# imalexlee/simple-vk-renderer

Measured on AMD Instinct MI355X. Metric: shaded fragments/s, higher is better.
Workload: dtype f32

## Files before the change

### simple-vk-renderer_amd/csrc/k_image.hip

```cpp
#include <hip/hip_fp16.h>

#include "svr_launch.h"

namespace svr {

__global__ __launch_bounds__(256) void fill16f_kernel(uint4* dst, uint32_t n_vec, uint32_t n_pixels, uint2 px, const uint32_t* poison) {
  if (*poison) return;
  for (uint32_t i = blockIdx.x * blockDim.x + threadIdx.x; i < n_vec; i += gridDim.x * blockDim.x)
    dst[i] = make_uint4(px.x, px.y, px.x, px.y);
  if (blockIdx.x == 0 && threadIdx.x == 0 && (n_pixels & 1u))
    reinterpret_cast<uint2*>(dst)[n_pixels - 1] = px;
}
__global__ __launch_bounds__(256) void fill8_kernel(uint32_t* dst, uint32_t n_pixels, uint32_t px, const uint32_t* poison) {
  if (*poison) return;
  uint32_t n_vec = n_pixels >> 2;
  uint4* d4 = reinterpret_cast<uint4*>(dst);
  for (uint32_t i = blockIdx.x * blockDim.x + threadIdx.x; i < n_vec; i += gridDim.x * blockDim.x)
    d4[i] = make_uint4(px, px, px, px);
  if (blockIdx.x == 0 && threadIdx.x < (n_pixels & 3u)) dst[(n_vec << 2) + threadIdx.x] = px;
}

static inline uint32_t stream_grid(uint32_t n_items) {
  uint32_t g = (n_items + 255u) / 256u;
  return g < 1u ? 1u : (g > 2048u ? 2048u : g);
}

void launch_fill_color(void* color, uint32_t n_pixels, int color_format, uint64_t packed_pixel, const uint32_t* poison,
                       hipStream_t s) {
  if (color_format == SVR_COLOR_RGBA16F) {
    uint2 px = make_uint2((uint32_t)packed_pixel, (uint32_t)(packed_pixel >> 32));
    uint32_t n_vec = n_pixels >> 1;
    hipLaunchKernelGGL(fill16f_kernel, dim3(stream_grid(n_vec)), dim3(256), 0, s, (uint4*)color, n_vec, n_pixels, px, poison);
  } else {
    hipLaunchKernelGGL(fill8_kernel, dim3(stream_grid(n_pixels >> 2)), dim3(256), 0, s, (uint32_t*)color, n_pixels,
                       (uint32_t)packed_pixel, poison);
  }
}

__global__ __launch_bounds__(256) void downsample_kernel(const uint32_t* src, uint32_t sw, uint32_t sh, uint32_t* dst,
                                                         uint32_t dw, uint32_t dh) {
  uint32_t idx = blockIdx.x * blockDim.x + threadIdx.x;
  if (idx >= dw * dh) return;
  uint32_t i = idx % dw, j = idx / dw;
  long long nx = (long long)(2u * i + 1u) * sw - dw, dx = 2ll * dw;
  long long ny = (long long)(2u * j + 1u) * sh - dh, dy = 2ll * dh;
  long long i0 = nx >= 0 ? nx / dx : -((-nx + dx - 1) / dx);
  long long j0 = ny >= 0 ? ny / dy : -((-ny + dy - 1) / dy);
  long long wx1 = nx - i0 * dx, wx0 = dx - wx1;
  long long wy1 = ny - j0 * dy, wy0 = dy - wy1;
  long long i1 = i0 + 1, j1 = j0 + 1;
  i0 = min(max(i0, 0ll), (long long)sw - 1);
  i1 = min(max(i1, 0ll), (long long)sw - 1);
  j0 = min(max(j0, 0ll), (long long)sh - 1);
  j1 = min(max(j1, 0ll), (long long)sh - 1);
  uint32_t t00 = src[j0 * sw + i0], t10 = src[j0 * sw + i1], t01 = src[j1 * sw + i0], t11 = src[j1 * sw + i1];
  long long den = dx * dy;
  uint32_t out = 0;
#pragma unroll
  for (int c = 0; c < 4; c++) {
    long long a = (t00 >> (8 * c)) & 0xffu, b = (t10 >> (8 * c)) & 0xffu;
    long long cc = (t01 >> (8 * c)) & 0xffu, d = (t11 >> (8 * c)) & 0xffu;
    long long num = wy0 * (wx0 * a + wx1 * b) + wy1 * (wx0 * cc + wx1 * d);
    long long q = num / den, r = num - q * den;
    if (2 * r > den || (2 * r == den && (q & 1))) q++;
    out |= (uint32_t)q << (8 * c);
  }
  dst[idx] = out;
}

void launch_downsample(const uint8_t* src, uint32_t sw, uint32_t sh, uint8_t* dst, uint32_t dw, uint32_t dh,
                       hipStream_t s) {
  uint32_t n = dw * dh;
  hipLaunchKernelGGL(downsample_kernel, dim3((n + 255u) / 256u), dim3(256), 0, s, (const uint32_t*)src, sw, sh,
                     (uint32_t*)dst, dw, dh);
}

__device__ __forceinline__ uint32_t h2un8(uint32_t hbits) {
  float f = __half2float(__ushort_as_half((unsigned short)hbits));
  return (uint32_t)__float2int_rn(fminf(fmaxf(f, 0.0f), 1.0f) * 255.0f);
}
__global__ __launch_bounds__(256) void cvt16f_to_8_kernel(const uint2* src, uint32_t* dst, uint32_t n_pixels) {
  for (uint32_t i = blockIdx.x * blockDim.x + threadIdx.x; i < n_pixels; i += gridDim.x * blockDim.x) {
    uint2 p = src[i];
    dst[i] = h2un8(p.x & 0xffffu) | (h2un8(p.x >> 16) << 8) | (h2un8(p.y & 0xffffu) << 16) | (h2un8(p.y >> 16) << 24);
  }
}
__device__ __forceinline__ float pin32(float x) {
  asm volatile("" : "+v"(x));
  return x;
}
__device__ __forceinline__ void store_target(void* color, int fmt, size_t p, float r, float g, float b, float a) {
  if (fmt == SVR_COLOR_RGBA16F) {
    r = pin32(r); g = pin32(g); b = pin32(b); a = pin32(a);
    uint32_t hr = __half_as_ushort(__float2half_rn(r)), hg = __half_as_ushort(__float2half_rn(g));
    uint32_t hb = __half_as_ushort(__float2half_rn(b)), ha = __half_as_ushort(__float2half_rn(a));
    reinterpret_cast<uint2*>(color)[p] = make_uint2(hr | (hg << 16), hb | (ha << 16));
  } else {
    auto un8 = [](float f) { return (uint32_t)__float2int_rn(fminf(fmaxf(f, 0.0f), 1.0f) * 255.0f); };
    reinterpret_cast<uint32_t*>(color)[p] = un8(r) | (un8(g) << 8) | (un8(b) << 16) | (un8(a) << 24);
  }
}

__device__ __forceinline__ float sky_cos(float x) {
  const float kTwoOverPi = 0x1.45f306p-1f, kPio2Hi = 0x1.921fb6p+0f, kPio2Mid = -0x1.777a5cp-25f, kPio2Lo = -0x1.ee59dap-50f;
  float k = rintf(x * kTwoOverPi);
  float r = fmaf(-k, kPio2Hi, x);
  r = fmaf(-k, kPio2Mid, r);
  r = fmaf(-k, kPio2Lo, r);
  float z = r * r;
  float sn = fmaf(fmaf(fmaf(-1.9515295891e-4f, z, 8.3321608736e-3f), z, -1.6666654611e-1f) * z, r, r);
  float cs = fmaf(fmaf(fmaf(2.443315711809948e-5f, z, -1.388731625493765e-3f), z, 4.166664568298827e-2f) * z, z,
                  fmaf(-0.5f, z, 1.0f));
  int q = (int)k & 3;
  float v = (q & 1) ? sn : cs;
  return (q == 1 || q == 2) ? -v : v;
}
__device__ __forceinline__ float sky_fract(float a) { return a - floorf(a); }
__device__ __forceinline__ float sky_noisy_star(float x, float y, float thr) {
  float s = sky_fract(415.92653f * (sky_cos(x * 37.0f) + sky_cos(y * 57.0f)));
  if (!(s >= thr)) return 0.0f;
  float t = (s - thr) / (1.0f - thr);
  float t2 = t * t, t4 = t2 * t2;
  return t4 * t2;
}

struct BackgroundData {
  float d[16];
};
__global__ __launch_bounds__(256) void background_kernel(void* color, int fmt, uint32_t W, uint32_t H, uint32_t y_first,
                                                         uint32_t n_rows, int effect, BackgroundData pc, const uint32_t* poison) {
  if (*poison) return;
  const float fh = (float)H;
  const uint32_t n = W * n_rows;
  for (uint32_t i = blockIdx.x * blockDim.x + threadIdx.x; i < n; i += gridDim.x * blockDim.x) {
    uint32_t x = i % W, y = y_first + i / W;
    float r, g, b, a;
    if (effect == SVR_BACKGROUND_GRADIENT) {
      float blend = (float)y / fh, inv = 1.0f - blend;
      r = fmaf(pc.d[4], blend, pc.d[0] * inv);
      g = fmaf(pc.d[5], blend, pc.d[1] * inv);
      b = fmaf(pc.d[6], blend, pc.d[2] * inv);
      a = fmaf(pc.d[7], blend, pc.d[3] * inv);
    } else {
      float fx = (float)x, fy = (float)y, thr = pc.d[3];
      float sx = fx + 0.2f, sy = fy + -0.06f;
      float frx = sky_fract(sx), fry = sky_fract(sy), gx = floorf(sx), gy = floorf(sy);
      float v1 = sky_noisy_star(gx, gy, thr), v2 = sky_noisy_star(gx, gy + 1.0f, thr);
      float v3 = sky_noisy_star(gx + 1.0f, gy, thr), v4 = sky_noisy_star(gx + 1.0f, gy + 1.0f, thr);
      float star = (v1 * (1.0f - frx)) * (1.0f - fry);
      star = fmaf(v2 * (1.0f - frx), fry, star);
      star = fmaf(v3 * frx, 1.0f - fry, star);
      star = fmaf(v4 * frx, fry, star);
      r = (pc.d[0] * fy) / fh + star;
      g = (pc.d[1] * fy) / fh + star;
      b = (pc.d[2] * fy) / fh + star;
      a = 1.0f;
    }
// ... 109 lines not shown
```

### simple-vk-renderer_amd/csrc/k_tile.hip

```cpp
#include <hip/hip_fp16.h>

#include <hip/hip_ext.h>

#include <cstdlib>
#include <type_traits>

#include "svr_launch.h"

namespace svr {

constexpr uint32_t REC_COMMON = 0x80000000u;
#ifndef SVR_PRIO_COST
#define SVR_PRIO_COST 200u
#endif
constexpr int BATCH = 64;
constexpr uint32_t SREC = 7;

constexpr float kInv255 = 0x1.010102p-8f;
constexpr float kG0 = 0x1.c51282p-2f, kG1 = -0x1.14a3a2p-2f, kG2 = 0x1.37536ap-3f, kG3 = -0x1.778474p-5f;

__device__ __forceinline__ float lod_from_rho2(float rho2) {
  uint32_t bits = f2u(rho2);
  int e = (int)(bits >> 23) - 127;
  float m = u2f((bits & 0x7fffffu) | 0x3f800000u);
  float t = m - 1.0f;
  float g = fmaf(fmaf(fmaf(kG3, t, kG2), t, kG1), t, kG0);
  float s = t * (1.0f - t);
  float l = fmaf(s, g, t);
  float lam = 0.5f * ((float)e + l);
  lam = (rho2 <= 0x1p+100f) ? lam : 50.0f;
  lam = (rho2 >= 0x1p-100f) ? lam : -50.0f;
  return lam;
}

__device__ __forceinline__ float lerpf(float a, float b, float t) { return fmaf(t, b - a, a); }

struct TexD {
  uint32_t base_off;
  uint32_t w, h, lw, lh, levels, filters;
  float min_lod, max_lod;
};

struct Taps {
  uint32_t o00, o10, o01, o11;
  float alpha, beta;
};
template <bool POW2 = false>
__device__ __forceinline__ Taps level_taps(int wl, int hl, uint32_t base, bool linear, float u, float v) {
  float U = (u - floorf(u)) * (float)wl;
  float V = (v - floorf(v)) * (float)hl;
  float Uh = U - 0.5f, Vh = V - 0.5f;
  float fu = floorf(linear ? Uh : U), fv = floorf(linear ? Vh : V);
  Taps tp;
  tp.alpha = linear ? Uh - fu : 0.0f;
  tp.beta = linear ? Vh - fv : 0.0f;
  int i0 = (int)fu, j0 = (int)fv;
  int i1 = linear ? i0 + 1 : i0, j1 = linear ? j0 + 1 : j0;
  if (POW2) {
    i0 &= wl - 1;
    i1 &= wl - 1;
    j0 &= hl - 1;
    j1 &= hl - 1;
  } else {
    if (i0 < 0) i0 += wl;
    if (i0 >= wl) i0 -= wl;
    if (i1 >= wl) i1 -= wl;
    if (j0 < 0) j0 += hl;
    if (j0 >= hl) j0 -= hl;
    if (j1 >= hl) j1 -= hl;
  }
  const uint32_t r0 = __umul24((uint32_t)j0, (uint32_t)wl), r1 = __umul24((uint32_t)j1, (uint32_t)wl);
  tp.o00 = base + (r0 + (uint32_t)i0) * 4u;
  tp.o10 = base + (r0 + (uint32_t)i1) * 4u;
  tp.o01 = base + (r1 + (uint32_t)i0) * 4u;
  tp.o11 = base + (r1 + (uint32_t)i1) * 4u;
  return tp;
}
__device__ __forceinline__ uint32_t texel(const uint8_t* arena, uint32_t off) {
  return *reinterpret_cast<const uint32_t*>(arena + off);
}
__device__ __forceinline__ float chan(uint32_t t, int c) { return (float)((t >> (8 * c)) & 0xffu) * kInv255; }
__device__ __forceinline__ float bilerp(uint32_t t00, uint32_t t10, uint32_t t01, uint32_t t11, int c, float a, float b) {
  return lerpf(lerpf(chan(t00, c), chan(t10, c), a), lerpf(chan(t01, c), chan(t11, c), a), b);
}

__device__ __forceinline__ float interp3(float a0, float da1, float da2, float b1, float b2, float r) {
  return fmaf(b2, da2, fmaf(b1, da1, a0)) * r;
}

struct FragAttr {
  float b1, b2, r, u, v, nx, ny, nz, light, cr, cg, cb, won;
};

__device__ __forceinline__ float quad_partner_x(float v) { return u2f((uint32_t)__builtin_amdgcn_mov_dpp((int)f2u(v), 0xB1, 0xf, 0xf, true)); }
__device__ __forceinline__ float quad_partner_y(float v) { return u2f((uint32_t)__builtin_amdgcn_mov_dpp((int)f2u(v), 0x128, 0xf, 0xf, true)); }
template <bool TRACE, bool COMMON = false, bool ATTR = false>
__device__ __forceinline__ float4 shade_pixel(const FrameParams& P, uint32_t rec, int px, int py, float* trace, const bool quads = false,
                                              FragAttr* fa = nullptr) {
  const TriRec* tr = P.recs + rec;
  const uint4* q4 = reinterpret_cast<const uint4*>(tr);
  const float4* f4 = reinterpret_cast<const float4*>(tr);
  const double2* d2 = reinterpret_cast<const double2*>(tr);
  uint4 hdr = q4[0];
  float4 zrow = f4[1];
  double2 c2 = d2[2], c3 = d2[3], c4 = d2[4], c5 = d2[5], c6 = d2[6];
  uint4 td = q4[7];
  float4 s0 = f4[8], s1 = f4[9], s2 = f4[10], s3 = f4[11], s4 = f4[12], s5 = f4[13], s6 = f4[14];
  uint32_t flags = hdr.w;
  float inv_area = zrow.w;
  double A1, B1, A2, B2, e1, e2;
  double C1 = c5.y, C2 = c6.x;
  A1 = c2.y; B1 = c4.x; A2 = c3.x; B2 = c4.y;
  double dx = (double)px, dy = (double)py;
  e1 = fma(A1, dx, fma(B1, dy, C1)) + ((flags & F_T1) ? 1.0 : 0.0);
  e2 = fma(A2, dx, fma(B2, dy, C2)) + ((flags & F_T2) ? 1.0 : 0.0);
  TexD t;
  t.base_off = (uint32_t)(unsigned long long)__double_as_longlong(c6.y);
  t.w = td.x & 0xffffu;
  t.h = td.x >> 16;
  t.lw = td.y & 0xffu;
  t.lh = (td.y >> 8) & 0xffu;
  t.levels = (td.y >> 16) & 0xffu;
  t.filters = td.y >> 24;
  t.min_lod = u2f(td.z);
  t.max_lod = u2f(td.w);
  float b1 = (float)e1 * inv_area, b2 = (float)e2 * inv_area;
  float q0 = s0.x, dq1 = s0.y, dq2 = s0.z;
  const float qq = fmaf(b2, dq2, fmaf(b1, dq1, q0));
  float hb1 = 0.0f, hb2 = 0.0f, vb1 = 0.0f, vb2 = 0.0f, hq = 1.0f, vq = 1.0f;
  if (!quads) {
    double sxp = (px & 1) ? -1.0 : 1.0, syp = (py & 1) ? -1.0 : 1.0;
    hb1 = (float)fma(sxp, A1, e1) * inv_area, hb2 = (float)fma(sxp, A2, e2) * inv_area;
    vb1 = (float)fma(syp, B1, e1) * inv_area, vb2 = (float)fma(syp, B2, e2) * inv_area;
    hq = fmaf(hb2, dq2, fmaf(hb1, dq1, q0)), vq = fmaf(vb2, dq2, fmaf(vb1, dq1, q0));
  }
  float r, hr = 0.0f, vr = 0.0f;
  if (COMMON && !quads) {
    rcp3_ieee(qq, hq, vq, r, hr, vr);
  } else {
    r = rcp_ieee(qq);
  }
  const uint32_t kind = COMMON ? (uint32_t)PIPE_MESH : ((flags >> F_KIND_SHIFT) & 3u);
  float cr = interp3(s1.z, s3.z, s5.z, b1, b2, r);
  float cg = interp3(s1.w, s3.w, s5.w, b1, b2, r);
  float cb = interp3(s2.x, s4.x, s6.x, b1, b2, r);
  if (ATTR) { fa->b1 = b1; fa->b2 = b2; fa->r = r; fa->won = 1.0f; }
  if (kind == PIPE_COLORED_TRIANGLE) return make_float4(cr, cg, cb, 1.0f);
  float u = interp3(s2.y, s4.y, s6.y, b1, b2, r), v = interp3(s2.z, s4.z, s6.z, b1, b2, r);
  if (ATTR) { fa->u = u; fa->v = v; }
  if (!COMMON) {
    hr = rcp_ieee(hq);
    vr = rcp_ieee(vq);
  }
  float uh, vh, uv_, vv_;
  if (quads) {
    uh = quad_partner_x(u), vh = quad_partner_x(v);
    uv_ = quad_partner_y(u), vv_ = quad_partner_y(v);
  } else {
    uh = interp3(s2.y, s4.y, s6.y, hb1, hb2, hr), vh = interp3(s2.z, s4.z, s6.z, hb1, hb2, hr);
    uv_ = interp3(s2.y, s4.y, s6.y, vb1, vb2, vr), vv_ = interp3(s2.z, s4.z, s6.z, vb1, vb2, vr);
  }
  float dudx = (px & 1) ? (u - uh) : (uh - u);
  float dvdx = (px & 1) ? (v - vh) : (vh - v);
  float dudy = (py & 1) ? (u - uv_) : (uv_ - u);
  float dvdy = (py & 1) ? (v - vv_) : (vv_ - v);
  float W0 = (float)t.w, H0 = (float)t.h;
  float mx = dudx * W0, my = dvdx * H0;
  float nx_ = dudy * W0, ny_ = dvdy * H0;
  float rho2 = fmaxf(fmaf(mx, mx, my * my), fmaf(nx_, nx_, ny_ * ny_));
  float lambda = fminf(fmaxf(lod_from_rho2(rho2), t.min_lod), t.max_lod);
  const bool linear = COMMON ? true : (((lambda <= 0.0f) ? (t.filters & 1u) : ((t.filters >> 1) & 1u)) != 0u);
  int q = (int)t.levels - 1;
  const bool mip_linear = COMMON ? true : (((t.filters >> 2) & 1u) != 0u);
  int dn = min(max((int)ceilf(lambda + 0.5f) - 1, 0), q);
  float lc = fminf(fmaxf(lambda, 0.0f), (float)q);
  float fl = floorf(lc);
  int dhi = mip_linear ? (int)fl : dn;
  float delta = mip_linear ? lc - fl : 0.0f;
  int dlo = mip_linear ? min(dhi + 1, q) : dn;
  float us = (fabsf(u) < 8388608.0f) ? u : 0.0f, vs = (fabsf(v) < 8388608.0f) ? v : 0.0f;
  const int whi = (int)max(t.w >> dhi, 1u), hhi = (int)max(t.h >> dhi, 1u);
  const uint32_t bhi = t.base_off + mip_offset(t.lw, t.lh, (uint32_t)dhi);
  Taps th = level_taps<COMMON>(whi, hhi, bhi, linear, us, vs);
  const uint8_t* tb = P.tex_arena;
  uint32_t h00 = texel(tb, th.o00), h10 = texel(tb, th.o10), h01 = texel(tb, th.o01), h11 = texel(tb, th.o11);
  const bool two_levels = __any(delta != 0.0f);
  Taps tl = th;
  uint32_t l00 = 0, l10 = 0, l01 = 0, l11 = 0;
  if (two_levels) {
    const int wlo = (int)max(t.w >> dlo, 1u), hlo = (int)max(t.h >> dlo, 1u);
    const uint32_t step = 4u << ((uint32_t)max((int)t.lw - dhi, 0) + (uint32_t)max((int)t.lh - dhi, 0));
    const uint32_t blo = dlo != dhi ? bhi + step : bhi;
    tl = level_taps<COMMON>(wlo, hlo, blo, linear, us, vs);
    l00 = texel(tb, tl.o00);
    l10 = texel(tb, tl.o10);
    l01 = texel(tb, tl.o01);
    l11 = texel(tb, tl.o11);
  }
  float4 tx;
  tx.x = bilerp(h00, h10, h01, h11, 0, th.alpha, th.beta);
  tx.y = bilerp(h00, h10, h01, h11, 1, th.alpha, th.beta);
  tx.z = bilerp(h00, h10, h01, h11, 2, th.alpha, th.beta);
  tx.w = 1.0f;
  if (two_levels) {
    tx.x = lerpf(tx.x, bilerp(l00, l10, l01, l11, 0, tl.alpha, tl.beta), delta);
    tx.y = lerpf(tx.y, bilerp(l00, l10, l01, l11, 1, tl.alpha, tl.beta), delta);
    tx.z = lerpf(tx.z, bilerp(l00, l10, l01, l11, 2, tl.alpha, tl.beta), delta);
  }
  if (TRACE) {
    trace[0] = (float)(hdr.z >> 2); trace[1] = b1; trace[2] = b2; trace[3] = r; trace[4] = u; trace[5] = v;
    trace[6] = dudx; trace[7] = dvdx; trace[8] = dudy; trace[9] = dvdy; trace[10] = lambda;
    trace[11] = tx.x; trace[12] = tx.y; trace[13] = tx.z;
    trace[26] = hb1; trace[27] = hb2; trace[28] = vb1; trace[29] = vb2; trace[30] = hr; trace[31] = vr;
  }
  if (kind == PIPE_TEX_IMAGE) {
    tx.w = bilerp(h00, h10, h01, h11, 3, th.alpha, th.beta);
    if (two_levels) tx.w = lerpf(tx.w, bilerp(l00, l10, l01, l11, 3, tl.alpha, tl.beta), delta);
    return tx;
  }
  float nx = interp3(s0.w, s2.w, s4.w, b1, b2, r);
  float ny = interp3(s1.x, s3.x, s5.x, b1, b2, r);
  float nz = interp3(s1.y, s3.y, s5.y, b1, b2, r);
  const float* L = P.scene.sunlight_direction;
  float d = fmaf(nz, L[2], fmaf(ny, L[1], nx * L[0]));
  float light = fmaxf(d, 0.1f);
  float sunw = P.scene.sunlight_color[3];
  cr = cr * tx.x;
  cg = cg * tx.y;
  cb = cb * tx.z;
  float4 o;
  o.x = fmaf(cr * light, sunw, cr * P.scene.ambient_color[0]);
  o.y = fmaf(cg * light, sunw, cg * P.scene.ambient_color[1]);
  o.z = fmaf(cb * light, sunw, cb * P.scene.ambient_color[2]);
  o.w = 1.0f;
  if (TRACE) {
    trace[15] = nx; trace[16] = ny; trace[17] = nz; trace[18] = cr; trace[19] = cg; trace[20] = cb;
    trace[21] = light; trace[22] = o.x; trace[23] = o.y; trace[24] = o.z; trace[25] = o.w;
  }
  if (ATTR) { fa->nx = nx; fa->ny = ny; fa->nz = nz; fa->light = light; fa->cr = cr; fa->cg = cg; fa->cb = cb; }
  return o;
}

template <int FMT>
struct Codec;
template <>
struct Codec<SVR_COLOR_RGBA16F> {
  typedef uint2 enc_t;
  static __device__ __forceinline__ float pin(float x) {
    asm volatile("" : "+v"(x));
    return x;
  }
  static __device__ __forceinline__ enc_t encode(float4 c) {
    c.x = pin(c.x); c.y = pin(c.y); c.z = pin(c.z); c.w = pin(c.w);
    uint32_t r = __half_as_ushort(__float2half_rn(c.x)), g = __half_as_ushort(__float2half_rn(c.y));
    uint32_t b = __half_as_ushort(__float2half_rn(c.z)), a = __half_as_ushort(__float2half_rn(c.w));
    return make_uint2(r | (g << 16), b | (a << 16));
  }
  static __device__ __forceinline__ float4 decode(enc_t e) {
    return make_float4(__half2float(__ushort_as_half((unsigned short)(e.x & 0xffffu))),
                       __half2float(__ushort_as_half((unsigned short)(e.x >> 16))),
                       __half2float(__ushort_as_half((unsigned short)(e.y & 0xffffu))),
                       __half2float(__ushort_as_half((unsigned short)(e.y >> 16))));
  }
};
template <>
struct Codec<SVR_COLOR_RGBA8> {
  typedef uint32_t enc_t;
  static __device__ __forceinline__ uint32_t un8(float f) {
    return (uint32_t)__float2int_rn(fminf(fmaxf(f, 0.0f), 1.0f) * 255.0f);
  }
  static __device__ __forceinline__ enc_t encode(float4 c) {
    return un8(c.x) | (un8(c.y) << 8) | (un8(c.z) << 16) | (un8(c.w) << 24);
  }
  static __device__ __forceinline__ float4 decode(enc_t e) {
    return make_float4(chan(e, 0), chan(e, 1), chan(e, 2), chan(e, 3));
  }
// ... 1340 lines not shown
```

### simple-vk-renderer_amd/csrc/svr_api.hip

```cpp
#include <hip/hip_runtime.h>

#include <algorithm>
#include <chrono>
#include <cmath>
#include <cstdio>
#include <cstring>
#include <deque>
#include <memory>
#include <numeric>
#include <string>
#include <type_traits>
#include <utility>
#include <vector>

#include "../../include/svr_depth.h"
#include "../../include/svr_draw_list.h"
#include "../../include/svr_attributes.h"
#include "../../include/svr_ids.h"
#include "../../include/svr_lighting.h"
#include "../../include/svr_post.h"
#include "../../include/svr_temporal.h"
#include "../../include/svr_ambient.h"
#include "../../include/svr_load.h"
#include "../../include/svr_occlusion.h"
// ... 1129 lines not shown
  if (!ctx || !out || (!indices && n_indices) || (!vertices && n_vertices))
    return fail(SVR_ERR_INVALID_ARGUMENT, "svr_upload_mesh: null argument");
  if (n_vertices > 0xffffffffull || n_indices > 0xffffffffull)
    return fail(SVR_ERR_UNSUPPORTED, "svr_upload_mesh: more than 2^32 elements");
  for (size_t i = 0; i < n_indices; i++)
    if (indices[i] >= n_vertices) return fail(SVR_ERR_INVALID_ARGUMENT, "svr_upload_mesh: index out of range");
  if (int e = use_device(ctx)) return e;
  MeshRes m;
  DEV_ALLOC(m.vtx, std::max<size_t>(n_vertices * sizeof(SvrVertex), 64));
  hipError_t r = dev_alloc(m.idx, std::max<size_t>(n_indices * 4, 64));
  if (r != hipSuccess) return fail(SVR_ERR_OUT_OF_MEMORY, std::string("hipMalloc(indices): ") + hipGetErrorString(r));
  if (n_vertices) HIPCHK(hipMemcpy(m.vtx.get(), vertices, n_vertices * sizeof(SvrVertex), hipMemcpyHostToDevice));
  if (n_indices) HIPCHK(hipMemcpy(m.idx.get(), indices, n_indices * 4, hipMemcpyHostToDevice));
  {
    const size_t n_groups = (n_indices + GROUP_INDICES - 1) / GROUP_INDICES;
    std::vector<float> boxes(std::max<size_t>(n_groups, 1) * GROUP_WORDS);
    for (size_t g = 0; g < n_groups; g++) {
      float lo[3] = {INFINITY, INFINITY, INFINITY}, hi[3] = {-INFINITY, -INFINITY, -INFINITY};
      uint32_t vmin = 0xffffffffu, vmax = 0u;
      const size_t end = std::min(n_indices, (g + 1) * GROUP_INDICES);
      for (size_t i = g * GROUP_INDICES; i < end; i++) {
        vmin = std::min(vmin, indices[i]);
        vmax = std::max(vmax, indices[i]);
        const float* p = vertices[indices[i]].position;
        for (int k = 0; k < 3; k++) {
          lo[k] = p[k] < lo[k] ? p[k] : lo[k];
          hi[k] = p[k] > hi[k] ? p[k] : hi[k];
          if (!std::isfinite(p[k])) lo[k] = hi[k] = NAN;
        }
      }
      for (int k = 0; k < 3; k++) {
        boxes[g * GROUP_WORDS + k] = lo[k];
        boxes[g * GROUP_WORDS + 3 + k] = hi[k];
      }
      std::memcpy(&boxes[g * GROUP_WORDS + 6], &vmin, 4);
      std::memcpy(&boxes[g * GROUP_WORDS + 7], &vmax, 4);
    }
    hipError_t rg = dev_alloc(m.groups, boxes.size() * sizeof(float));
    if (rg == hipSuccess) rg = hipMemcpy(m.groups.get(), boxes.data(), boxes.size() * sizeof(float), hipMemcpyHostToDevice);
    if (rg != hipSuccess) return fail(SVR_ERR_OUT_OF_MEMORY, std::string("svr_upload_mesh: index-group boxes: ") + hipGetErrorString(rg));
  }
  m.n_vtx = n_vertices;
  m.n_idx = n_indices;
  m.alive = true;
  ctx->meshes.push_back(std::move(m));
  *out = (SvrMesh)ctx->meshes.size();
  return SVR_OK;
}

int svr_destroy_mesh(SvrContext* ctx, SvrMesh mesh) {
  MeshRes* m = ctx ? get_mesh(ctx, mesh) : nullptr;
  if (!m) return fail(SVR_ERR_BAD_HANDLE, "svr_destroy_mesh: bad handle");
  if (int e = use_device(ctx)) return e;
  if (int e = finish_pending(ctx)) return e;
  m->vtx.reset();
  m->idx.reset();
  m->groups.reset();
  m->alive = false;
  ctx->mesh_epoch++;
  return SVR_OK;
}

int svr_create_image(SvrContext* ctx, const void* rgba8, uint32_t width, uint32_t height, int mipmapped,
                     SvrImage* out) {
  if (!ctx || !rgba8 || !out) return fail(SVR_ERR_INVALID_ARGUMENT, "svr_create_image: null argument");
  if (width == 0 || height == 0 || width > 16384 || height > 16384)
    return fail(SVR_ERR_INVALID_ARGUMENT, "svr_create_image: extent must be in 1..16384");
  if (int e = use_device(ctx)) return e;
  ImageRes im;
  im.w = width;
  im.h = height;
  im.levels = 1;
  if (mipmapped) {
    uint32_t m = std::max(width, height);
    while (m > 1) {
      m >>= 1;
      im.levels++;
    }
  }
  while ((1u << im.lw) < width) im.lw++;
  while ((1u << im.lh) < height) im.lh++;
  for (uint32_t l = 0; l < im.levels; l++) im.off[l] = mip_offset(im.lw, im.lh, l);
  uint32_t lw = width, lh = height;
  size_t total = (size_t)mip_offset(im.lw, im.lh, im.levels - 1) +
                 (size_t)std::max(1u, width >> (im.levels - 1)) * std::max(1u, height >> (im.levels - 1)) * 4;
  if (im.lw + im.lh > 28) return fail(SVR_ERR_UNSUPPORTED, "svr_create_image: image larger than 1 GiB");
  im.bytes = std::max<size_t>(total, 256);
  if (int e = arena_alloc(ctx, im.bytes, &im.arena_off)) return e;
  uint8_t* base = ctx->tex_arena.get() + im.arena_off;
  hipError_t r = hipMemcpy(base, rgba8, (size_t)width * height * 4, hipMemcpyHostToDevice);
  if (r != hipSuccess) {
    arena_free(ctx, im.arena_off, im.bytes);
    return fail(SVR_ERR_DEVICE, std::string("hipMemcpy(image): ") + hipGetErrorString(r));
  }
  lw = width;
  lh = height;
  for (uint32_t l = 1; l < im.levels; l++) {
    uint32_t dw = std::max(1u, lw >> 1), dh = std::max(1u, lh >> 1);
    launch_downsample(base + im.off[l - 1], lw, lh, base + im.off[l], dw, dh, ctx->stream);
    lw = dw;
    lh = dh;
  }
  HIPCHK(hipGetLastError());
  HIPCHK(hipStreamSynchronize(ctx->stream));
  im.alive = true;
  ctx->images.push_back(im);
  *out = (SvrImage)ctx->images.size();
  return SVR_OK;
}

int svr_destroy_image(SvrContext* ctx, SvrImage image) {
  ImageRes* im = ctx ? get_image(ctx, image) : nullptr;
  if (!im) return fail(SVR_ERR_BAD_HANDLE, "svr_destroy_image: bad handle");
  if (int e = use_device(ctx)) return e;
  if (int e = finish_pending(ctx)) return e;
  arena_free(ctx, im->arena_off, im->bytes);
  im->alive = false;
  return SVR_OK;
}

int svr_read_image_level(SvrContext* ctx, SvrImage image, uint32_t level, void* dst, size_t bytes, uint32_t* w,
                         uint32_t* h) {
  ImageRes* im = ctx ? get_image(ctx, image) : nullptr;
  if (!im) return fail(SVR_ERR_BAD_HANDLE, "svr_read_image_level: bad handle");
  if (level >= im->levels) return fail(SVR_ERR_INVALID_ARGUMENT, "svr_read_image_level: no such level");
  uint32_t lw = std::max(1u, im->w >> level), lh = std::max(1u, im->h >> level);
  if (w) *w = lw;
  if (h) *h = lh;
  if (dst) {
    size_t need = (size_t)lw * lh * 4;
    if (bytes < need) return fail(SVR_ERR_INVALID_ARGUMENT, "svr_read_image_level: buffer too small");
    if (int e = use_device(ctx)) return e;
    HIPCHK(hipMemcpy(dst, ctx->tex_arena.get() + im->arena_off + im->off[level], need, hipMemcpyDeviceToHost));
  }
  return SVR_OK;
}

int svr_create_sampler(SvrContext* ctx, const SvrSamplerDesc* desc, SvrSampler* out) {
  if (!ctx || !desc || !out) return fail(SVR_ERR_INVALID_ARGUMENT, "svr_create_sampler: null argument");
  if ((desc->mag_filter | 1) != 1 || (desc->min_filter | 1) != 1 || (desc->mipmap_mode | 1) != 1)
    return fail(SVR_ERR_INVALID_ARGUMENT, "svr_create_sampler: bad filter enum");
  if (!(desc->min_lod <= desc->max_lod)) return fail(SVR_ERR_INVALID_ARGUMENT, "svr_create_sampler: min_lod > max_lod");
  ctx->samplers.push_back(*desc);
  *out = (SvrSampler)ctx->samplers.size();
  return SVR_OK;
}

int svr_write_material(SvrContext* ctx, int pass, const float color_factors[4], const float metal_rough_factors[4],
                       SvrImage color_image, SvrSampler color_sampler, SvrMaterial* out) {
  if (!ctx || !color_factors || !out) return fail(SVR_ERR_INVALID_ARGUMENT, "svr_write_material: null argument");
  if (!get_image(ctx, color_image)) return fail(SVR_ERR_BAD_HANDLE, "svr_write_material: bad image");
  if (color_sampler == 0 || color_sampler > ctx->samplers.size())
    return fail(SVR_ERR_BAD_HANDLE, "svr_write_material: bad sampler");
  if (pass < 0 || pass > 2) return fail(SVR_ERR_INVALID_ARGUMENT, "svr_write_material: bad pass");
  if (int e = use_device(ctx)) return e;
  MaterialRes m;
  m.pass = pass;
  for (int i = 0; i < 4; i++) {
    m.cf[i] = color_factors[i];
    m.mr[i] = metal_rough_factors ? metal_rough_factors[i] : 0.0f;
  }
  m.image = color_image - 1;
  m.sampler = color_sampler - 1;
  ctx->materials.push_back(m);
  ctx->tex_slots = 0;
  *out = (SvrMaterial)ctx->materials.size();
  return SVR_OK;
}

static uint64_t encode_clear(const SvrContext* ctx, const float rgba[4]) {
  uint64_t packed;
  if (ctx->fmt == SVR_COLOR_RGBA16F) {
    packed = (uint64_t)host_f32_to_f16(rgba[0]) | ((uint64_t)host_f32_to_f16(rgba[1]) << 16) |
             ((uint64_t)host_f32_to_f16(rgba[2]) << 32) | ((uint64_t)host_f32_to_f16(rgba[3]) << 48);
  } else {
    packed = 0;
    for (int k = 0; k < 4; k++) {
      float c = rgba[k];
      if (!(c == c)) c = 0.0f;
      c = c < 0.0f ? 0.0f : (c > 1.0f ? 1.0f : c);
      packed |= (uint64_t)(uint32_t)std::nearbyintf(c * 255.0f) << (8 * k);
    }
  }
  return packed;
}

int svr_clear_color(SvrContext* ctx, const float rgba[4]) {
  if (!ctx || !rgba) return fail(SVR_ERR_INVALID_ARGUMENT, "svr_clear_color: null argument");
  if (int e = use_device(ctx)) return e;
  if (int e = poll_pending(ctx)) return e;
  const uint64_t packed = encode_clear(ctx, rgba);
  if (int e = flush_clear(ctx)) return e;
  ctx->pending_clear.valid = true;
  ctx->pending_clear.target = ctx->color;
  ctx->pending_clear.y0 = ctx->sy;
  ctx->pending_clear.rows = ctx->sh;
  ctx->pending_clear.fmt = ctx->fmt;
  ctx->pending_clear.packed = packed;
  if (ctx->tuning & TUNE_NO_LAZY_CLEAR) return flush_clear(ctx);
  return SVR_OK;
}

int svr_draw_background(SvrContext* ctx, int effect, const float data[16]) {
  if (!ctx || !data) return fail(SVR_ERR_INVALID_ARGUMENT, "svr_draw_background: null argument");
  if (effect != SVR_BACKGROUND_GRADIENT && effect != SVR_BACKGROUND_SKY)
    return fail(SVR_ERR_INVALID_ARGUMENT, "svr_draw_background: unknown effect");
  if (int e = use_device(ctx)) return e;
  if (int e = poll_pending(ctx)) return e;
  if (int e = flush_clear(ctx)) return e;
  SvrContext::LoggedOp* op = nullptr;
  if (int e = log_fill(ctx, SvrContext::OpKind::Background, ctx->color, ctx->fmt, ctx->sy, ctx->sh, &op)) return e;
  op->bg_effect = effect;
  std::memcpy(op->bg_data, data, sizeof(op->bg_data));
  return submit_fill(ctx, *op);
}

// ... 1237 lines not shown
```

### simple-vk-renderer_amd/csrc/svr_device.h

```cpp
#pragma once

#include <hip/hip_runtime.h>
#include <stdint.h>

#include "../../include/svr.h"

namespace svr {

constexpr int TILE = 32;
constexpr int TILE_SHIFT = 5;
constexpr int WAVE = 64;
constexpr float GUARD = 16384.0f;
constexpr uint32_t NO_REC = 0xffffffffu;
#ifndef SVR_RCP_VARIANT
#define SVR_RCP_VARIANT 1
#endif

enum PipelineKind : uint32_t { PIPE_MESH = 0, PIPE_COLORED_TRIANGLE = 1, PIPE_TEX_IMAGE = 2 };

constexpr uint32_t F_T1 = 1u;
constexpr uint32_t F_T2 = 2u;
constexpr uint32_t F_KIND_SHIFT = 4;
constexpr uint32_t F_TRANSPARENT = 256u;
constexpr uint32_t F_VIEW_SHIFT = 24;
constexpr uint32_t MAX_VIEWS = 16;

constexpr uint32_t TUNE_NO_TILE_ORDER = 1u;
constexpr uint32_t TUNE_NO_LAZY_CLEAR = 4u;
constexpr uint32_t TUNE_NO_PIPELINE = 2u;
constexpr uint32_t TUNE_NO_SPLIT = 8u;
constexpr uint32_t TUNE_HIZ = 64u;
constexpr uint32_t TUNE_NO_HIZ = 32u;
constexpr uint32_t TUNE_NO_POLL = 16u;

constexpr uint32_t SPLIT_MAX = 256;
constexpr uint32_t SPLIT_EXTRA = 4 * SPLIT_MAX;
constexpr uint32_t SPLIT_MIN_COST = 100;
constexpr uint32_t SPLIT_TILES_MAX = 4096;
constexpr uint32_t ROW_COST_MAX = 512;
#ifndef SVR_AB_TILE_SLOTS
#define SVR_AB_TILE_SLOTS 1024
#endif
constexpr uint32_t TILE_SLOTS = SVR_AB_TILE_SLOTS;
__host__ __device__ inline uint32_t tile_cost(uint32_t n_op, uint32_t n_tr) { return 40u + (n_op >> 3) + n_tr - (n_tr >> 2); }
constexpr uint32_t SPLIT_SORT_MAX = 1392;

struct DrawDesc {
  float mat[16];
  float mvp[16];
  float color_factors[4];
  const SvrVertex* vtx;
  const uint32_t* idx;
  uint32_t tri_count;
  uint32_t tri_base;
  uint32_t tex;
  uint32_t flags;
  const float* groups;
  uint32_t first_index;
  uint32_t pad;
};
static_assert(sizeof(DrawDesc) == 192 && offsetof(DrawDesc, vtx) == 144 && offsetof(DrawDesc, groups) == 176, "DrawDesc layout");
constexpr uint32_t GROUP_INDICES = 192;
__host__ __device__ inline uint32_t chunk_phase(uint32_t first_index) { return first_index % 3u == 0u ? (first_index / 3u) & 63u : 0u; }
__host__ __device__ inline uint32_t chunk_count(uint32_t first_index, uint32_t tri_count) {
  return tri_count ? (chunk_phase(first_index) + tri_count + 63u) / 64u : 0u;
}
__host__ __device__ inline uint32_t chunk_first(uint32_t first_index, uint32_t k) { return k ? 64u * k - chunk_phase(first_index) : 0u; }
__host__ __device__ inline uint32_t chunk_len(uint32_t first_index, uint32_t tri_count, uint32_t first_tri) {
  const uint32_t to_grid = 64u - ((chunk_phase(first_index) + first_tri) & 63u), left = tri_count - first_tri;
  return to_grid < left ? to_grid : left;
}
constexpr uint32_t GROUP_WORDS = 8;

struct WaveChunk {
  uint32_t draw;
  uint32_t first_tri;
};

struct TexBinding {
  uint32_t base_off;
  uint32_t pad0;
  uint32_t wh;
  uint32_t info;
  float min_lod, max_lod;
  uint32_t pad[2];
};
static_assert(sizeof(TexBinding) == 32, "TexBinding layout");

__host__ __device__ inline uint32_t mip_offset(uint32_t lw, uint32_t lh, uint32_t level) {
  const uint32_t a = lw < lh ? lw : lh, b = lw < lh ? lh : lw;
  const uint32_t l1 = level < a ? level : a;
  const uint32_t ones = l1 ? (0x55555555u >> (32u - 2u * l1)) : 0u;
  uint32_t off = ones << ((lw + lh + 4u - 2u * l1) & 31u);
  if (level > a) off += 4u * ((1u << (b - a + 1u)) - (1u << (b - level + 1u)));
  return off;
}

struct TriRec {
  int16_t minx, miny, maxx, maxy;
  uint32_t key;
  uint32_t flags;
  float z0, dz1, dz2, inv_area;
  double A[3], B[3], C[3];
  uint32_t tex_off, tex_pad;
  uint32_t tex_wh, tex_info;
  float tex_min_lod, tex_max_lod;
  float q0, dq1, dq2;
  float a0[8], da1[8], da2[8];
  float pad2;
  uint32_t object, primitive;
  float pad3[2];
};
static_assert(sizeof(TriRec) == 256, "TriRec layout");
static_assert(offsetof(TriRec, object) == 240, "TriRec layout: the ID words are piece 15's x and y");
constexpr uint32_t REC_ID_PIECE = offsetof(TriRec, object) / 16u;
static_assert(offsetof(TriRec, A) == 32 && offsetof(TriRec, tex_off) == 104 && offsetof(TriRec, tex_wh) == 112 &&
                  offsetof(TriRec, q0) == 128, "TriRec layout");

struct ClipItem {
  uint32_t draw;
  uint32_t tri;
};

struct Counters {
  uint32_t n_clip;
  uint32_t n_extra;
  uint32_t total_entries;
  uint32_t overflow;
  unsigned long long rasterized;
  unsigned long long shaded;
  unsigned long long binned;
  uint32_t n_big;
  uint32_t n_pairs;
  uint32_t n_pairs_rest;
  uint32_t sort_used;
  uint32_t n_split;
  uint32_t cost_sum;
  uint32_t flat_draws;
  uint32_t flat_tris;
  uint32_t flat_chunks;
  uint32_t flat_culled;
  uint32_t hiz_bad;
  uint32_t occl_tested;
  uint32_t occl_culled;
  uint32_t occl_tris;
};
static_assert(sizeof(Counters) == 96, "Counters layout");

struct MeshEntry {
  const SvrVertex* vtx;
  const uint32_t* idx;
  const float* groups;
  uint64_t pad;
};
struct MatEntry {
  float cf[4];
  uint32_t pass;
  uint32_t pad[3];
};

constexpr uint32_t PYR_MAX_LEVELS = 14;

struct FrameParams {
  void* color;
  float* depth;
  uint32_t W, H;
  uint32_t sx, sy, sw, sh;
  uint32_t tiles_x, tiles_y, n_tiles;
  uint32_t rstride, roff;
  uint32_t depth_load;
  const DrawDesc* draws;
  const WaveChunk* chunks;
  uint32_t n_chunks;
  uint32_t n_tris;
  TriRec* recs;
  uint32_t extra_cap;
  ClipItem* clip_queue;
  uint32_t clip_cap;
  uint32_t* big_queue;
// ... 341 lines not shown
```

### simple-vk-renderer_amd/csrc/svr_launch.h

```cpp
#pragma once
#include "../../include/svr_ambient.h"
#include "../../include/svr_lighting.h"
#include "../../include/svr_post.h"
#include "../../include/svr_temporal.h"
#include "svr_device.h"

namespace svr {

void launch_prologue(const void* host_src, void* dst, size_t copy_bytes, void* zero, size_t zero_bytes, uint32_t n_draws,
                     const SvrSceneData& scene, hipStream_t s);
void launch_setup(const FrameParams& P, bool depth_only, hipStream_t s);
void launch_mesh_vert(const SvrVertex* vtx, uint32_t first, uint32_t n, const float* world16,
                      const float* viewproj16, const float* color_factors4, float* out_clip,
                      float* out_varyings, hipStream_t s);
void launch_vertex_shader(const SvrVertex* vtx, uint32_t first, uint32_t n, const float* matrix16, float* out_clip,
                          float* out_varyings, hipStream_t s);
void launch_flatten(const FlattenParams& F, hipStream_t s);
void launch_list_flatten(const FlattenParams& F, hipStream_t s);
void launch_bin_count(const FrameParams& P, hipStream_t s);
void launch_bin_scan(const FrameParams& P, hipStream_t s);
void launch_bin_fill(const FrameParams& P, hipStream_t s, hipEvent_t done);
void launch_tiles(const FrameParams& P, int color_format, bool count_fragments, bool depth_only, hipStream_t s, hipEvent_t done);
void launch_fill_color(void* color, uint32_t n_pixels, int color_format, uint64_t packed_pixel, const uint32_t* poison,
                       hipStream_t s);
void launch_background(void* color, int color_format, uint32_t W, uint32_t H, uint32_t y_first, uint32_t n_rows, int effect,
                       const float data[16], const uint32_t* poison, hipStream_t s);
void launch_blit(const void* color, int color_format, uint32_t W, uint32_t H, void* dst, uint32_t dw, uint32_t dh, uint32_t row_first,
                 uint32_t n_rows, int dst_format, const uint32_t* poison, uint32_t rstride, uint32_t roff, uint32_t row_end, uint32_t* status,
                 uint32_t status_ok, hipStream_t s);
void launch_downsample(const uint8_t* src, uint32_t sw, uint32_t sh, uint8_t* dst, uint32_t dw, uint32_t dh,
                       hipStream_t s);
void launch_rgba16f_to_rgba8(const void* src, void* dst, uint32_t n_pixels, hipStream_t s);
uint32_t pyramid_levels(uint32_t W, uint32_t H);
size_t pyramid_offsets(uint32_t W, uint32_t H, uint32_t* off);
void launch_pyramid(const float* depth, uint32_t W, uint32_t H, uint32_t* pyr, const uint32_t* off, uint32_t n_levels,
                    const uint32_t* poison, hipStream_t s);
struct LightLaunch {
  void* color;
  const float* depth;
  const float4* normal;
  const float4* albedo;
  uint32_t W, H;
  uint32_t sx, sy, sw, sh;
  uint32_t tiles_x, rstride, roff;
  float two_over_w, two_over_h;
  float inv_viewproj[16];
  float ambient_color[4], sunlight_direction[4], sunlight_color[4];
  const SvrPointLight* lights;
  uint32_t n_lights;
  const float* shadow_depth;
  uint32_t shadow_w, shadow_h;
  float shadow_half_w, shadow_half_h;
  float shadow_viewproj[16];
  float shadow_bias;
  uint32_t* tile_counts;
  const uint32_t* poison;
  const float* ao;
};
void launch_light(const LightLaunch& L, int color_format, uint32_t tiles_y, hipStream_t s);
struct PostLaunch {
  uint2* color;
  uint32_t W;
  uint32_t sx, sy, sw, sh;
  uint2* levels;
  uint32_t n_levels;
  uint32_t off[SVR_POST_MAX_LEVELS], lw[SVR_POST_MAX_LEVELS], lh[SVR_POST_MAX_LEVELS];
  float exposure, threshold, intensity;
  uint32_t tonemap;
  const uint32_t* poison;
};
size_t post_level_layout(uint32_t sw, uint32_t sh, uint32_t n_levels, uint32_t* off, uint32_t* lw, uint32_t* lh);
void launch_post(const PostLaunch& P, hipStream_t s);
struct TemporalLaunch {
  uint2* color;
  const float* depth;
  uint32_t W, H;
  uint32_t sx, sy, sw, sh;
  const uint2* hist_in;
  uint2* hist_out;
  uint32_t history_valid;
  uint32_t clamp;
  float reproject[16];
  float blend;
  float two_over_w, two_over_h;
  float half_w, half_h;
  const uint32_t* poison;
};
void launch_temporal(const TemporalLaunch& A, hipStream_t s);
struct AmbientLaunch {
  const float* depth;
  const float4* normal;
  float2* raw;
  float* out;
  uint32_t W, H;
  uint32_t sx, sy, sw, sh;
  float inv_viewproj[16];
  float two_over_w, two_over_h;
  float radius_px;
  float radius2;
  float bias;
  float coef;
  float sharpness;
  uint32_t blur;
  const uint32_t* poison;
};
void launch_ambient(const AmbientLaunch& A, hipStream_t s);
void launch_rcp_sweep(int variant, unsigned long long first, unsigned long long count, unsigned long long* out19, hipStream_t s);

}
```

Before: 44.72 billion.

## Store texture mip levels in 8x4 texel tiles for better sampling locality

```diff
diff --git a/simple-vk-renderer_amd/csrc/k_image.hip b/simple-vk-renderer_amd/csrc/k_image.hip
--- a/simple-vk-renderer_amd/csrc/k_image.hip
+++ b/simple-vk-renderer_amd/csrc/k_image.hip
@@ -37,8 +37,8 @@
   }
 }
 
-__global__ __launch_bounds__(256) void downsample_kernel(const uint32_t* src, uint32_t sw, uint32_t sh, uint32_t* dst,
-                                                         uint32_t dw, uint32_t dh) {
+__global__ __launch_bounds__(256) void downsample_kernel(const uint32_t* src, uint32_t sw, uint32_t sh, uint32_t splw, uint32_t* dst,
+                                                         uint32_t dw, uint32_t dh, uint32_t dplw) {
   uint32_t idx = blockIdx.x * blockDim.x + threadIdx.x;
   if (idx >= dw * dh) return;
   uint32_t i = idx % dw, j = idx / dw;
@@ -53,7 +53,8 @@
   i1 = min(max(i1, 0ll), (long long)sw - 1);
   j0 = min(max(j0, 0ll), (long long)sh - 1);
   j1 = min(max(j1, 0ll), (long long)sh - 1);
-  uint32_t t00 = src[j0 * sw + i0], t10 = src[j0 * sw + i1], t01 = src[j1 * sw + i0], t11 = src[j1 * sw + i1];
+  auto at = [&](long long x, long long y) { return src[texel_offset(splw, (uint32_t)x, (uint32_t)y) >> 2]; };
+  uint32_t t00 = at(i0, j0), t10 = at(i1, j0), t01 = at(i0, j1), t11 = at(i1, j1);
   long long den = dx * dy;
   uint32_t out = 0;
 #pragma unroll
@@ -65,14 +66,29 @@
     if (2 * r > den || (2 * r == den && (q & 1))) q++;
     out |= (uint32_t)q << (8 * c);
   }
-  dst[idx] = out;
-}
-
-void launch_downsample(const uint8_t* src, uint32_t sw, uint32_t sh, uint8_t* dst, uint32_t dw, uint32_t dh,
-                       hipStream_t s) {
+  dst[texel_offset(dplw, i, j) >> 2] = out;
+}
+
+void launch_downsample(const uint8_t* src, uint32_t sw, uint32_t sh, uint32_t splw, uint8_t* dst, uint32_t dw, uint32_t dh,
+                       uint32_t dplw, hipStream_t s) {
   uint32_t n = dw * dh;
-  hipLaunchKernelGGL(downsample_kernel, dim3((n + 255u) / 256u), dim3(256), 0, s, (const uint32_t*)src, sw, sh,
-                     (uint32_t*)dst, dw, dh);
+  hipLaunchKernelGGL(downsample_kernel, dim3((n + 255u) / 256u), dim3(256), 0, s, (const uint32_t*)src, sw, sh, splw,
+                     (uint32_t*)dst, dw, dh, dplw);
+}
+
+template <bool TO_TILED>
+__global__ __launch_bounds__(256) void retile_kernel(uint32_t* linear, uint32_t* tiled, uint32_t w, uint32_t h, uint32_t plw) {
+  const uint32_t n = w * h;
+  for (uint32_t idx = blockIdx.x * blockDim.x + threadIdx.x; idx < n; idx += gridDim.x * blockDim.x) {
+    const uint32_t t = texel_offset(plw, idx % w, idx / w) >> 2;
+    if (TO_TILED) tiled[t] = linear[idx];
+    else linear[idx] = tiled[t];
+  }
+}
+void launch_retile(bool to_tiled, void* linear, uint8_t* tiled, uint32_t w, uint32_t h, uint32_t plw, hipStream_t s) {
+  const dim3 grid(stream_grid(w * h)), block(256);
+  if (to_tiled) hipLaunchKernelGGL(retile_kernel<true>, grid, block, 0, s, (uint32_t*)linear, (uint32_t*)tiled, w, h, plw);
+  else hipLaunchKernelGGL(retile_kernel<false>, grid, block, 0, s, (uint32_t*)linear, (uint32_t*)tiled, w, h, plw);
 }
 
 __device__ __forceinline__ uint32_t h2un8(uint32_t hbits) {
diff --git a/simple-vk-renderer_amd/csrc/k_tile.hip b/simple-vk-renderer_amd/csrc/k_tile.hip
--- a/simple-vk-renderer_amd/csrc/k_tile.hip
+++ b/simple-vk-renderer_amd/csrc/k_tile.hip
@@ -46,7 +46,7 @@
   float alpha, beta;
 };
 template <bool POW2 = false>
-__device__ __forceinline__ Taps level_taps(int wl, int hl, uint32_t base, bool linear, float u, float v) {
+__device__ __forceinline__ Taps level_taps(int wl, int hl, uint32_t plw, uint32_t base, bool linear, float u, float v) {
   float U = (u - floorf(u)) * (float)wl;
   float V = (v - floorf(v)) * (float)hl;
   float Uh = U - 0.5f, Vh = V - 0.5f;
@@ -69,11 +69,12 @@
     if (j0 >= hl) j0 -= hl;
     if (j1 >= hl) j1 -= hl;
   }
-  const uint32_t r0 = __umul24((uint32_t)j0, (uint32_t)wl), r1 = __umul24((uint32_t)j1, (uint32_t)wl);
-  tp.o00 = base + (r0 + (uint32_t)i0) * 4u;
-  tp.o10 = base + (r0 + (uint32_t)i1) * 4u;
-  tp.o01 = base + (r1 + (uint32_t)i0) * 4u;
-  tp.o11 = base + (r1 + (uint32_t)i1) * 4u;
+  const uint32_t x0 = texel_offset_x((uint32_t)i0), x1 = texel_offset_x((uint32_t)i1);
+  const uint32_t y0 = base + texel_offset_y(plw, (uint32_t)j0), y1 = base + texel_offset_y(plw, (uint32_t)j1);
+  tp.o00 = y0 + x0;
+  tp.o10 = y0 + x1;
+  tp.o01 = y1 + x0;
+  tp.o11 = y1 + x1;
   return tp;
 }
 __device__ __forceinline__ uint32_t texel(const uint8_t* arena, uint32_t off) {
@@ -181,7 +182,7 @@
   float us = (fabsf(u) < 8388608.0f) ? u : 0.0f, vs = (fabsf(v) < 8388608.0f) ? v : 0.0f;
   const int whi = (int)max(t.w >> dhi, 1u), hhi = (int)max(t.h >> dhi, 1u);
   const uint32_t bhi = t.base_off + mip_offset(t.lw, t.lh, (uint32_t)dhi);
-  Taps th = level_taps<COMMON>(whi, hhi, bhi, linear, us, vs);
+  Taps th = level_taps<COMMON>(whi, hhi, level_lw(t.lw, (uint32_t)dhi), bhi, linear, us, vs);
   const uint8_t* tb = P.tex_arena;
   uint32_t h00 = texel(tb, th.o00), h10 = texel(tb, th.o10), h01 = texel(tb, th.o01), h11 = texel(tb, th.o11);
   const bool two_levels = __any(delta != 0.0f);
@@ -189,9 +190,9 @@
   uint32_t l00 = 0, l10 = 0, l01 = 0, l11 = 0;
   if (two_levels) {
     const int wlo = (int)max(t.w >> dlo, 1u), hlo = (int)max(t.h >> dlo, 1u);
-    const uint32_t step = 4u << ((uint32_t)max((int)t.lw - dhi, 0) + (uint32_t)max((int)t.lh - dhi, 0));
+    const uint32_t step = level_bytes(t.lw, t.lh, (uint32_t)dhi);
     const uint32_t blo = dlo != dhi ? bhi + step : bhi;
-    tl = level_taps<COMMON>(wlo, hlo, blo, linear, us, vs);
+    tl = level_taps<COMMON>(wlo, hlo, level_lw(t.lw, (uint32_t)dlo), blo, linear, us, vs);
     l00 = texel(tb, tl.o00);
     l10 = texel(tb, tl.o10);
     l01 = texel(tb, tl.o01);
diff --git a/simple-vk-renderer_amd/csrc/svr_api.hip b/simple-vk-renderer_amd/csrc/svr_api.hip
--- a/simple-vk-renderer_amd/csrc/svr_api.hip
+++ b/simple-vk-renderer_amd/csrc/svr_api.hip
@@ -1235,22 +1235,25 @@
   while ((1u << im.lh) < height) im.lh++;
   for (uint32_t l = 0; l < im.levels; l++) im.off[l] = mip_offset(im.lw, im.lh, l);
   uint32_t lw = width, lh = height;
-  size_t total = (size_t)mip_offset(im.lw, im.lh, im.levels - 1) +
-                 (size_t)std::max(1u, width >> (im.levels - 1)) * std::max(1u, height >> (im.levels - 1)) * 4;
   if (im.lw + im.lh > 28) return fail(SVR_ERR_UNSUPPORTED, "svr_create_image: image larger than 1 GiB");
+  const size_t total = (size_t)mip_offset(im.lw, im.lh, im.levels - 1) + level_bytes(im.lw, im.lh, im.levels - 1);
   im.bytes = std::max<size_t>(total, 256);
+  const size_t linear = (size_t)width * height * 4;
+  DevPtr<uint8_t> staging;
+  if (dev_alloc(staging, linear) != hipSuccess) return fail(SVR_ERR_OUT_OF_MEMORY, "svr_create_image: staging buffer");
   if (int e = arena_alloc(ctx, im.bytes, &im.arena_off)) return e;
   uint8_t* base = ctx->tex_arena.get() + im.arena_off;
-  hipError_t r = hipMemcpy(base, rgba8, (size_t)width * height * 4, hipMemcpyHostToDevice);
+  hipError_t r = hipMemcpy(staging.get(), rgba8, linear, hipMemcpyHostToDevice);
   if (r != hipSuccess) {
     arena_free(ctx, im.arena_off, im.bytes);
     return fail(SVR_ERR_DEVICE, std::string("hipMemcpy(image): ") + hipGetErrorString(r));
   }
+  launch_retile(true, staging.get(), base, width, height, level_lw(im.lw, 0), ctx->stream);
   lw = width;
   lh = height;
   for (uint32_t l = 1; l < im.levels; l++) {
     uint32_t dw = std::max(1u, lw >> 1), dh = std::max(1u, lh >> 1);
-    launch_downsample(base + im.off[l - 1], lw, lh, base + im.off[l], dw, dh, ctx->stream);
+    launch_downsample(base + im.off[l - 1], lw, lh, level_lw(im.lw, l - 1), base + im.off[l], dw, dh, level_lw(im.lw, l), ctx->stream);
     lw = dw;
     lh = dh;
   }
@@ -1284,7 +1287,12 @@
     size_t need = (size_t)lw * lh * 4;
     if (bytes < need) return fail(SVR_ERR_INVALID_ARGUMENT, "svr_read_image_level: buffer too small");
     if (int e = use_device(ctx)) return e;
-    HIPCHK(hipMemcpy(dst, ctx->tex_arena.get() + im->arena_off + im->off[level], need, hipMemcpyDeviceToHost));
+    DevPtr<uint8_t> staging;
+    if (dev_alloc(staging, need) != hipSuccess) return fail(SVR_ERR_OUT_OF_MEMORY, "svr_read_image_level: staging buffer");
+    launch_retile(false, staging.get(), ctx->tex_arena.get() + im->arena_off + im->off[level], lw, lh, level_lw(im->lw, level), ctx->stream);
+    HIPCHK(hipGetLastError());
+    HIPCHK(hipStreamSynchronize(ctx->stream));
+    HIPCHK(hipMemcpy(dst, staging.get(), need, hipMemcpyDeviceToHost));
   }
   return SVR_OK;
 }
diff --git a/simple-vk-renderer_amd/csrc/svr_device.h b/simple-vk-renderer_amd/csrc/svr_device.h
--- a/simple-vk-renderer_amd/csrc/svr_device.h
+++ b/simple-vk-renderer_amd/csrc/svr_device.h
@@ -87,14 +87,29 @@
 };
 static_assert(sizeof(TexBinding) == 32, "TexBinding layout");
 
+constexpr uint32_t TEX_TILE_LW = 3, TEX_TILE_LH = 2;
+constexpr uint32_t TEX_TILE_BYTES = 4u << (TEX_TILE_LW + TEX_TILE_LH);
+__host__ __device__ inline uint32_t level_lw(uint32_t lw, uint32_t level) { return lw > level + TEX_TILE_LW ? lw - level : TEX_TILE_LW; }
+__host__ __device__ inline uint32_t level_lh(uint32_t lh, uint32_t level) { return lh > level + TEX_TILE_LH ? lh - level : TEX_TILE_LH; }
+__host__ __device__ inline uint32_t level_bytes(uint32_t lw, uint32_t lh, uint32_t level) { return 4u << (level_lw(lw, level) + level_lh(lh, level)); }
+
 __host__ __device__ inline uint32_t mip_offset(uint32_t lw, uint32_t lh, uint32_t level) {
-  const uint32_t a = lw < lh ? lw : lh, b = lw < lh ? lh : lw;
-  const uint32_t l1 = level < a ? level : a;
+  const uint32_t cw = level_lw(lw, 0), ch = level_lh(lh, 0), nw = cw - TEX_TILE_LW, nh = ch - TEX_TILE_LH;
+  const uint32_t a = nw < nh ? nw : nh, b = nw < nh ? nh : nw;
+  const uint32_t l1 = level < a ? level : a, l2 = level < b ? level : b;
   const uint32_t ones = l1 ? (0x55555555u >> (32u - 2u * l1)) : 0u;
-  uint32_t off = ones << ((lw + lh + 4u - 2u * l1) & 31u);
-  if (level > a) off += 4u * ((1u << (b - a + 1u)) - (1u << (b - level + 1u)));
+  uint32_t off = ones << ((cw + ch + 4u - 2u * l1) & 31u);
+  if (level > a) off += (8u << (cw + ch - 2u * a)) - (8u << (cw + ch - a - l2));
+  if (level > b) off += (level - b) * TEX_TILE_BYTES;
   return off;
 }
+__host__ __device__ inline uint32_t texel_offset_x(uint32_t x) {
+  return ((x >> TEX_TILE_LW) << (TEX_TILE_LW + TEX_TILE_LH + 2u)) | ((x & ((1u << TEX_TILE_LW) - 1u)) << 2u);
+}
+__host__ __device__ inline uint32_t texel_offset_y(uint32_t plw, uint32_t y) {
+  return ((y >> TEX_TILE_LH) << (plw + TEX_TILE_LH + 2u)) | ((y & ((1u << TEX_TILE_LH) - 1u)) << (TEX_TILE_LW + 2u));
+}
+__host__ __device__ inline uint32_t texel_offset(uint32_t plw, uint32_t x, uint32_t y) { return texel_offset_x(x) + texel_offset_y(plw, y); }
 
 struct TriRec {
   int16_t minx, miny, maxx, maxy;
diff --git a/simple-vk-renderer_amd/csrc/svr_launch.h b/simple-vk-renderer_amd/csrc/svr_launch.h
--- a/simple-vk-renderer_amd/csrc/svr_launch.h
+++ b/simple-vk-renderer_amd/csrc/svr_launch.h
@@ -28,8 +28,9 @@
 void launch_blit(const void* color, int color_format, uint32_t W, uint32_t H, void* dst, uint32_t dw, uint32_t dh, uint32_t row_first,
                  uint32_t n_rows, int dst_format, const uint32_t* poison, uint32_t rstride, uint32_t roff, uint32_t row_end, uint32_t* status,
                  uint32_t status_ok, hipStream_t s);
-void launch_downsample(const uint8_t* src, uint32_t sw, uint32_t sh, uint8_t* dst, uint32_t dw, uint32_t dh,
-                       hipStream_t s);
+void launch_downsample(const uint8_t* src, uint32_t sw, uint32_t sh, uint32_t splw, uint8_t* dst, uint32_t dw, uint32_t dh,
+                       uint32_t dplw, hipStream_t s);
+void launch_retile(bool to_tiled, void* linear, uint8_t* tiled, uint32_t w, uint32_t h, uint32_t plw, hipStream_t s);
 void launch_rgba16f_to_rgba8(const void* src, void* dst, uint32_t n_pixels, hipStream_t s);
 uint32_t pyramid_levels(uint32_t W, uint32_t H);
 size_t pyramid_offsets(uint32_t W, uint32_t H, uint32_t* off);
```

Result: faster. 45.82 billion, median of 6 (+2.5%).
